# chenbinghui1/DSL

Hardware: AMD Instinct MI355X
Metric: imgs/sec training step, FCOS R50-FPN 1333x800 (higher is better)
Workload: dtype bf16; 1 GPU; FCOS R50-caffe-FPN supervised training step (BASELINE.json configs[1]), 2 x (3,800,1344) per GPU, synthetic COCO-shaped boxes, random-init weights; global_batch=2, parallelism=dp1, optimizer=SGD momentum 0.9 wd 1e-4

## Files before the change

dsl_amd/_lib.py:

```python
import ctypes as C
import os

import torch

HERE = os.path.dirname(os.path.abspath(__file__))
LIB_PATH = os.environ.get('DSL_HIP_LIB') or os.path.join(HERE, 'lib', 'libdsl_hip.so')
MAX_SEG = 5

if not os.path.exists(LIB_PATH):
    raise RuntimeError(
        f'{LIB_PATH} not found: the MI355X kernels are not built. Run `python -m dsl_amd.build` '
        '(needs hipcc); dsl_amd has no CPU or PyTorch fallback for its hot path.')
lib = C.CDLL(LIB_PATH)

I5 = C.c_int32 * MAX_SEG
F5 = C.c_float * MAX_SEG

CONV_RELU_OUT, CONV_RELU_IN, CONV_OUT_F32, CONV_MASK_FIRST, CONV_MASK_LAST, CONV_ADD_UPSAMPLE, \
    CONV_SMALL_C = 1, 2, 4, 8, 16, 32, 64
CONV_FP8 = 128
CONV_EPI_STAGED = 1 << 16
(OP_CONV, OP_WGRAD, OP_GN_FWD, OP_GN_BWD, OP_MAXPOOL, OP_SUM2X2, OP_COLSUM, OP_MEMSET, OP_PACK_IMAGE,
 OP_ASSIGN, OP_LOSS, OP_FORK, OP_JOIN, OP_WGRAD_GROUP, OP_RECORD, OP_WAIT) = range(1, 17)
OP_RLA = 17
OP_PACK_DGRAD = 18
OP_WGRAD_MULTI = 19
OP_PROF = 21
OP_QUANT_FP8, OP_QUANT_FP8_W, OP_FP8_COMB = 22, 23, 24
OP_FP8_PREP, OP_QUANT_FP8_DELAYED = 27, 28
OP_STEM_POOL = 25
OP_BNECK = 26
PROF_CLASSES = 8
MAX_MULTI = 16
SLOT_TAIL, SLOT_PREFIX = 13, 14
SLOT_PACKS = 15
SUMSQ_PARTS = 256
# ... 312 lines not shown
```

dsl_amd/csrc/conv.hip:

```cpp
#include <stdlib.h>
#include <algorithm>

#include <mutex>
#include <type_traits>
#include <vector>

#include "common.hpp"

namespace {

constexpr int BPX = 128;
constexpr int BK = 64;

struct ConvK {
  int nseg, n;
  int gh[DSL_MAX_SEG], gw[DSL_MAX_SEG], sh[DSL_MAX_SEG], sw[DSL_MAX_SEG];
  int dh[DSL_MAX_SEG], dw[DSL_MAX_SEG], ah[DSL_MAX_SEG], aw[DSL_MAX_SEG];
  int pxstart[DSL_MAX_SEG + 1];
  long long soff[DSL_MAX_SEG], doff[DSL_MAX_SEG], aoff[DSL_MAX_SEG];
  int cs, cd, ldd, lda, ldm, kh, kw, stride, pad, mode, os, flags;
  int lds;
  int ktiles, kc;
  int ident;
  int addfast;
// ... 10 lines not shown
  const uint16_t* addend;
  const uint16_t* mask;
  float* gnws;
  const uint16_t* gnx;
  const float* gngamma;
  const float* gnbeta;
  const float* gnstats;
};

#define CONV_HOT_PARAMS                                                                                                   \
  const uint16_t* h_wgt, const uint16_t* h_src, const int h_wrow, const int h_xcd_chunk, const int h_gx, const int h_gy, \
      const int h_splits, const int h_kt_per_split, const int h_ktiles, const int h_kc, const int h_kw, const int h_lds
#define CONV_HOT_ARGS(k) \
  (k).wgt, (k).src, (int)(k).wrow, (k).xcd_chunk, (k).gx, (k).gy, (k).splits, (k).kt_per_split, (k).ktiles, (k).kc, (k).kw, (k).lds

enum ConvGen { kGenV1 = 0, kGenGlds, kGenPipe, kGenPipeGn, kGenPipeSmallC, kGenF8, kNumConvGen };
struct ConvWaves { int wco, wpx; };
struct ConvTile {
  int bco, bpx, nst, occ;
  double eff;
  int prof;
  ConvWaves gen[kNumConvGen];
};
constexpr ConvTile kConvTiles[] = {
    {256, 192, 2, 1, 1.0,  1, {{}, {4, 2}, {4, 2}, {4, 2}, {},     {4, 2}}},
    {256, 128, 3, 1, 1.0,  2, {{}, {4, 2}, {4, 2}, {4, 2}, {},     {4, 2}}},
    {128, 256, 3, 1, 1.0,  2, {{}, {2, 4}, {2, 4}, {},     {},     {}}},
    {128, 128, 2, 2, 0.7,  0, {{}, {2, 2}, {2, 4}, {},     {},     {2, 4}}},
    {64,  256, 2, 2, 0.95, 2, {{}, {1, 4}, {1, 8}, {},     {1, 8}, {}}},
    {128, 64,  3, 2, 0.9,  2, {{}, {},     {2, 2}, {},     {},     {}}},
    {64,  64,  3, 3, 1.3,  2, {{}, {},     {1, 2}, {},     {},     {}}},
    {64,  128, 3, 2, 1.25, 2, {{}, {},     {1, 4}, {},     {},     {}}},
};
constexpr int kNumConvTiles = sizeof(kConvTiles) / sizeof(kConvTiles[0]);
constexpr size_t conv_lds_bytes(int bco, int bpx, int wpx, int nst, bool glds) {
  const size_t ring = (size_t)nst * (bco + bpx) * 128, stg = (size_t)32 * wpx * (bco * 4 + 16);
  return glds || ring > stg ? ring : stg;
}
constexpr size_t conv_lds_bytes(const ConvTile& t, int gen) { return conv_lds_bytes(t.bco, t.bpx, t.gen[gen].wpx, t.nst, gen == kGenGlds); }

__device__ __forceinline__ u32x4 relu_bf16x8(u32x4 v) {
#pragma unroll
  for (int i = 0; i < 4; ++i) {
    uint32_t w = v[i];
    uint32_t neg = (w >> 15) & 0x00010001u;
    v[i] = w & ~(neg * 0xffffu);
  }
// ... 32 lines not shown
  for (int s = 1; s < DSL_MAX_SEG; ++s) {
    const bool in = s < p.nseg && gp >= p.pxstart[s];
    ps = in ? p.pxstart[s] : ps;
    gh = in ? p.gh[s] : gh;
    gw = in ? p.gw[s] : gw;
    sh = in ? p.sh[s] : sh;
    sw = in ? p.sw[s] : sw;
    soff = in ? (int)p.soff[s] : soff;
  }
  const int q = gp - ps;
  const int hw = gh * gw;
  img = q / hw;
  const int rem = q - img * hw;
  y = rem / gw;
  x = rem - y * gw;
}

__device__ __forceinline__ void conv_epilogue4(const ConvK& p, long long dpix, long long apix, int co, float v[4]) {
  const bool out_f32 = (p.flags & DSL_CONV_OUT_F32) != 0;
  const bool relu_out = (p.flags & DSL_CONV_RELU_OUT) != 0;
  const bool mask_first = (p.flags & DSL_CONV_MASK_FIRST) != 0 && p.mask != nullptr;
  const bool mask_last = (p.flags & DSL_CONV_MASK_LAST) != 0 && p.mask != nullptr;
  const bool has_mask = mask_first || mask_last;
  if (co + 3 < p.cd) {
    if (p.scale) {
      const f32x4 s4 = *reinterpret_cast<const f32x4*>(p.scale + co);
#pragma unroll
      for (int e = 0; e < 4; ++e) v[e] *= s4[e];
    }
    if (p.bias) {
// ... 602 lines not shown
template <int NMF, int NDS, int NVM>
__device__ __forceinline__ void sched_stage() {
#pragma unroll
  for (int i = 0; i < NMF; ++i) {
    __builtin_amdgcn_sched_group_barrier(0x008, 1, 0);
    if (i < NDS) __builtin_amdgcn_sched_group_barrier(0x100, 1, 0);
    if (i < NVM) __builtin_amdgcn_sched_group_barrier(0x020, 1, 0);
  }
}

#ifdef DSL_TRACE_BUILD
constexpr int kTraceIters = 40;
__device__ unsigned long long g_conv_trace[8 * kTraceIters * 8 + 8 * 16 + 8];
#endif

template <int BCO, int BPX, int WCO, int WPX, int CT, int PT, int RING, bool GNB = false, class Stamp>
__device__ __forceinline__ void conv_tile_epilogue(const ConvK& p, f32x16 (&acc)[CT][PT], unsigned char* smem, const int co0, const int px0,
                                                   const int totpx, Stamp&& stamp) {
  constexpr int T = 64 * WCO * WPX;
  const int tid = threadIdx.x, lane = tid & 63;
  const int wave = __builtin_amdgcn_readfirstlane(tid >> 6);
  const int wave_co = wave / WPX, wave_px = wave % WPX;
  const int frow = lane & 31, fhalf = lane >> 5;
  constexpr int ROWB = BCO * 4 + 16;
  constexpr int CPX = 32 * WPX;
  constexpr int GPR = BCO / 8;
  static_assert(CPX * ROWB <= conv_lds_bytes(BCO, BPX, WPX, RING / ((BCO + BPX) * 128), false) &&
                conv_lds_bytes(BCO, BPX, WPX, RING / ((BCO + BPX) * 128), false) <= 160 * 1024,
                "epilogue staging must fit in LDS: the host sizes the launch's LDS with conv_lds_bytes, max(ring, staging)");
  static_assert(T % GPR == 0, "a thread keeps its channel group across the staged rows");
  const Affine8 aff = conv_affine8(p, co0 + (tid % GPR) * 8);
  const EpiFast ef = conv_epi_fast(p, co0 + (tid % GPR) * 8);
  constexpr int ROWH = BCO * 2 + 16;
  static_assert((long long)BPX * ROWH <= (long long)RING, "the bf16 tile fits in the ring");
  if ((ef.on || (p.addfast == 2 && !(p.flags & DSL_CONV_OUT_F32))) && ef.has_add && p.addfast && !ef.mask_first && !(ef.mask_last && ef.relu) &&
      (p.cd & 7) == 0) {
    constexpr int RB = BCO * 2;
    constexpr int NCH = RB / 16;
    constexpr int FSH = RB >= 256 ? 0 : (RB == 128 ? 1 : 2);
    static_assert((long long)BPX * RB <= (long long)RING, "the dense bf16 tile fits in the ring");
    static_assert((BPX * RB) % (T * 16) == 0, "whole DMA instructions per wave");
    constexpr int NDMA = BPX * RB / (T * 16);
    lds_barrier();
    {
      const __amdgpu_buffer_rsrc_t rs_add = __builtin_amdgcn_make_buffer_rsrc((void*)p.addend, 0, 0x7fffffff, 0x00020000);
#pragma unroll
      for (int i = 0; i < NDMA; ++i) {
        const int off = (i * (T / 64) + wave) * 1024 + lane * 16;
        const int row = off / RB, slot = (off % RB) >> 4;
        const int c = slot ^ ((row >> FSH) & (NCH - 1));
// ... 57 lines not shown
            u32x4 r = *reinterpret_cast<const u32x4*>(smem + row * RB + ((cgp ^ ((row >> FSH) & (NCH - 1))) << 4));
            if (ef.mask_last) {
              const u32x4 mm = *reinterpret_cast<const u32x4*>(ef.mask + (long long)gp * ef.ldm);
#pragma unroll
              for (int e = 0; e < 4; ++e)
                r[e] &= (bflo(mm[e]) > 0.f ? 0xffffu : 0x8000u) | (bfhi(mm[e]) > 0.f ? 0xffff0000u : 0x80000000u);
            }
            *reinterpret_cast<u32x4*>(out + (long long)gp * p.ldd) = r;
          }
        }
      }
    }
    stamp(3);
    return;
  }
  if (ef.on && !(p.flags & DSL_CONV_EPI_STAGED) && !ef.has_add && !ef.mask_first && !(ef.mask_last && ef.relu) && (p.cd & 7) == 0) {
    lds_barrier();
#pragma unroll
    for (int ct = 0; ct < CT; ++ct)
#pragma unroll
      for (int g = 0; g < 4; ++g) {
        const int col = wave_co * (32 * CT) + ct * 32 + 8 * g + 4 * fhalf;
        const bool in = co0 + col + 3 < p.cd;
        const f32x4 sc = (ef.has_scale && in) ? *reinterpret_cast<const f32x4*>(p.scale + co0 + col) : f32x4{1.f, 1.f, 1.f, 1.f};
        const f32x4 bi = (ef.has_bias && in) ? *reinterpret_cast<const f32x4*>(p.bias + co0 + col) : f32x4{0.f, 0.f, 0.f, 0.f};
#pragma unroll
        for (int pt = 0; pt < PT; ++pt) {
          float v[4];
#pragma unroll
          for (int j = 0; j < 4; ++j) {
            v[j] = acc[ct][pt][4 * g + j];
// ... 229 lines not shown
        f32x4 o = {acc[ct][pt][4 * g], acc[ct][pt][4 * g + 1], acc[ct][pt][4 * g + 2], acc[ct][pt][4 * g + 3]};
        *reinterpret_cast<f32x4*>(smem + (wave_px * 32 + frow) * ROWB + col * 4) = o;
      }
  };
  static_assert(PT <= 4, "slab dispatch");
#pragma nounroll
  for (int pt = 0; pt < PT; ++pt) {
    lds_barrier();
    stamp(1 + 3 * pt);
    if (pt == 0) stage_slab(std::integral_constant<int, 0>{});
    else if (pt == 1) stage_slab(std::integral_constant<int, (PT > 1 ? 1 : 0)>{});
    else if (pt == 2) stage_slab(std::integral_constant<int, (PT > 2 ? 2 : 0)>{});
    else stage_slab(std::integral_constant<int, (PT > 3 ? 3 : 0)>{});
    lds_barrier();
    stamp(2 + 3 * pt);
    if (ef.on && aff.full) {
      constexpr int NIT = CPX * GPR / T;
      static_assert(CPX * GPR % T == 0, "whole items per thread");
      const int pl0 = tid / GPR;
      const unsigned char* rd = smem + pl0 * ROWB + (tid % GPR) * 32;
#pragma nounroll
      for (int n_ = 0; n_ < NIT; ++n_) {
        const int pl = pl0 + n_ * (T / GPR);
        const int gp = px0 + (pl >> 5) * (32 * PT) + pt * 32 + (pl & 31);
        if (gp < totpx)
          conv_epilogue8_fast(ef, aff, gp, *reinterpret_cast<const f32x4*>(rd + n_ * (T / GPR) * ROWB),
                              *reinterpret_cast<const f32x4*>(rd + n_ * (T / GPR) * ROWB + 16));
      }
      stamp(3 + 3 * pt);
      continue;
    }
#pragma nounroll
    for (int id = tid; id < CPX * GPR; id += T) {
      const int pl = id / GPR, cg = id - pl * GPR;
      const int gp = px0 + (pl >> 5) * (32 * PT) + pt * 32 + (pl & 31);
      const int co = co0 + cg * 8;
      if (gp >= totpx || co >= p.cd) continue;
      const f32x4 lo = *reinterpret_cast<const f32x4*>(smem + pl * ROWB + cg * 32);
      const f32x4 hi = *reinterpret_cast<const f32x4*>(smem + pl * ROWB + cg * 32 + 16);
      float v[8] = {lo[0], lo[1], lo[2], lo[3], hi[0], hi[1], hi[2], hi[3]};
#ifdef DSL_ABLATE_BUILD
      if ((p.dbg & 512) && v[0] != 12345.678f) continue;
#endif
      long long dpix, apix;
      conv_out_index(p, gp, dpix, apix);
      conv_epilogue8a(p, dpix, apix, co, v, aff);
    }
    stamp(3 + 3 * pt);
  }
}

template <int BCO, int BPX, int WCO, int WPX, int NST, bool SMC = false, bool GNB = false>
__global__ __launch_bounds__(64 * WCO * WPX) void conv_pipe_kernel(CONV_HOT_PARAMS, const ConvK p) {
  extern __shared__ __attribute__((aligned(16))) unsigned char smem[];
  constexpr int T = 64 * WCO * WPX;
  constexpr int RPP = T / 8;
  constexpr int WPASS = BCO / RPP, XPASS = BPX / RPP;
  constexpr int TILE_W = BCO * 128;
  constexpr int STAGE = (BCO + BPX) * 128;
  constexpr int PT = BPX / WPX / 32;
  constexpr int CT = BCO / WCO / 32;
  constexpr int HB = 1;
  static_assert(BCO == WCO * CT * 32 && CT >= 1, "cout tiles per wave");
  static_assert(BCO % RPP == 0 && BPX % RPP == 0 && (BPX / WPX) % 32 == 0, "tile/thread mismatch");

  const int tid = threadIdx.x, lane = tid & 63;
  const int wave = __builtin_amdgcn_readfirstlane(tid >> 6);
// ... 7 lines not shown
  const int rem_t = wi - bz * (h_gx * h_gy);
  const int by = rem_t / h_gx;
  const int co0 = (rem_t - by * h_gx) * BCO;
  const int px0 = by * BPX;
  const int dt = tid, dwave = wave;
  const int lrow = dt >> 3;
  const int chunk = (dt & 7) ^ ((dt >> 4) & 7);

  const unsigned margin = (unsigned)(h_kw * h_lds * 2);
  const __amdgpu_buffer_rsrc_t rs_src =
      __builtin_amdgcn_make_buffer_rsrc((void*)(reinterpret_cast<const unsigned char*>(h_src) - margin), 0, 0x7fffffff, 0x00020000);
  const __amdgpu_buffer_rsrc_t rs_wgt = __builtin_amdgcn_make_buffer_rsrc((void*)h_wgt, 0, 0x7fffffff, 0x00020000);

  const int kt0 = bz * h_kt_per_split;
#ifdef DSL_ABLATE_BUILD
  const int kt1 = (p.dbg & 8) ? kt0 + 1 : min(kt0 + h_kt_per_split, h_ktiles);
#else
  const int kt1 = min(kt0 + h_kt_per_split, h_ktiles);
#endif
  const unsigned w_voff = (unsigned)(lrow * h_wrow + chunk * 8) * 2u;
  const unsigned w_pass = (unsigned)(RPP * h_wrow) * 2u;
  unsigned w_soff = (unsigned)(co0 * h_wrow + kt0 * BK) * 2u;
#pragma unroll
  for (int i = 0; i < WPASS; ++i) {
#ifdef DSL_ABLATE_BUILD
    if (p.dbg & 2) continue;
#endif
    __builtin_amdgcn_raw_ptr_buffer_load_lds(rs_wgt, (lptr_t)(smem + (i * RPP + dwave * 8) * 128), 16, w_voff, w_soff + i * w_pass, 0, 0);
  }
  __builtin_amdgcn_sched_barrier(0);

  const int totpx = p.pxstart[p.nseg];
  int cidx = kt0 % h_kc;
  int tap_r = (kt0 / h_kc) / h_kw, tap_s = (kt0 / h_kc) % h_kw;

  unsigned r_cur[XPASS], r_step[XPASS], r_mask[XPASS];
  int r_y[XPASS], r_x[XPASS], r_hw[XPASS];
#pragma unroll
  for (int i = 0; i < XPASS; ++i) {
    const int gp = px0 + lrow + RPP * i;
    int img, y, x, sh, sw, soff;
    const bool ok = gp < totpx;
    decode_pixel_src(p, ok ? gp : 0, img, y, x, sh, sw, soff);
    if (SMC) {
      r_y[i] = ok ? y * p.stride - p.pad : -100000;
      r_x[i] = x * p.stride - p.pad;
      r_hw[i] = (sh << 16) | sw;
      r_cur[i] = (unsigned)((soff + img * sh * sw + r_y[i] * sw + r_x[i]) * 16) + margin;
      r_step[i] = r_mask[i] = 0;
      continue;
    }
    const int row0 = p.mode == 0 ? y * p.stride - p.pad : y + p.pad;
    const int col0 = p.mode == 0 ? x * p.stride - p.pad : x + p.pad - (h_kw - 1);
    unsigned m = 0;
    for (int r = 0; r < p.kh; ++r) {
      const int sy = p.mode == 0 ? row0 + r : row0 - r;
      if (ok && (unsigned)sy < (unsigned)sh) m |= 1u << r;
// ... 8 lines not shown
    const unsigned base = (unsigned)((soff + img * sh * sw + row0 * sw + col0) * h_lds + chunk * 8) * 2u + margin;
    r_cur[i] = base + (unsigned)tap_r * r_step[i];
  }

  constexpr int LPT = WPASS + XPASS;
  constexpr int P0 = (LPT + 1) / 3;
  constexpr int P1 = P0 + (LPT - P0 + 1) / 2;
  int kt_next = kt0;
  unsigned t_sel = (1u << tap_r) | (0x100u << tap_s);
  unsigned t_soff = (unsigned)((p.mode == 0 ? tap_s : h_kw - 1 - tap_s) * h_lds * 2 + cidx * 128);
  unsigned t_wv = w_voff;
  int c_left = h_kc - cidx;
  unsigned r_v[XPASS];
#pragma unroll
  for (int i = 0; i < XPASS; ++i) r_v[i] = (r_mask[i] & t_sel) == t_sel ? r_cur[i] : 0x80000000u;
  auto pieces_of = [&](auto lo_c, auto hi_c, const unsigned ld_off, auto skipw_c) {
    constexpr int LO = decltype(lo_c)::value, HI = decltype(hi_c)::value;
    constexpr bool SKIPW = decltype(skipw_c)::value;
    unsigned char* stage = smem + ld_off;
    const bool live = kt_next < kt1;
    const unsigned s_off = t_soff;
    const unsigned wv = t_wv;
    int s_tr = 0, s_ts = 0;
    bool s_ok = false;
    if (SMC) {
      const int tap = kt_next * 8 + chunk;
      s_tr = tap / h_kw;
      s_ts = tap - s_tr * h_kw;
      s_ok = live && tap < p.kh * h_kw;
    }
// ... 13 lines not shown
          v = r_v[j];
          so = s_off;
        }
        __builtin_amdgcn_raw_ptr_buffer_load_lds(rs_src, (lptr_t)(stage + TILE_W + (j * RPP + dwave * 8) * 128), 16, v, so, 0, 0);
      } else if (!SKIPW) {
        const int i = j - XPASS;
        __builtin_amdgcn_raw_ptr_buffer_load_lds(rs_wgt, (lptr_t)(stage + (i * RPP + dwave * 8) * 128), 16, wv,
                                                 w_soff + i * w_pass, 0, 0);
      }
    }
    if (HI == LPT) {
      ++kt_next;
      w_soff += BK * 2;
      if (--c_left != 0) {
        t_soff += 128;
      } else {
        c_left = h_kc;
        const bool s_wrap = tap_s + 1 == h_kw;
        tap_s = s_wrap ? 0 : tap_s + 1;
        if (s_wrap) {
          ++tap_r;
#pragma unroll
          for (int i = 0; i < XPASS; ++i) r_cur[i] += r_step[i];
        }
        t_sel = (1u << tap_r) | (0x100u << tap_s);
        t_soff = (unsigned)((p.mode == 0 ? tap_s : h_kw - 1 - tap_s) * h_lds * 2);
#pragma unroll
        for (int i = 0; i < XPASS; ++i) r_v[i] = (r_mask[i] & t_sel) == t_sel ? r_cur[i] : 0x80000000u;
      }
      if (__builtin_expect(kt_next >= kt1, 0)) {
// ... 189 lines not shown
      if (gp >= totpx) continue;
      float* row = p.ws + ((long long)bz * totpx + gp) * p.cd_pad;
#pragma unroll
      for (int ct = 0; ct < CT; ++ct)
#pragma unroll
        for (int g = 0; g < 4; ++g) {
          const int co = co0 + wave_co * (32 * CT) + ct * 32 + 8 * g + 4 * (lane >> 5);
          f32x4 o = {acc[ct][pt][4 * g], acc[ct][pt][4 * g + 1], acc[ct][pt][4 * g + 2], acc[ct][pt][4 * g + 3]};
          *reinterpret_cast<f32x4*>(row + co) = o;
        }
    }
    return;
  }

#ifdef DSL_TRACE_BUILD
  conv_tile_epilogue<BCO, BPX, WCO, WPX, CT, PT, NST * STAGE, GNB>(p, acc, smem, co0, px0, totpx, [&](int i_) { TRE(i_); });
#else
  conv_tile_epilogue<BCO, BPX, WCO, WPX, CT, PT, NST * STAGE, GNB>(p, acc, smem, co0, px0, totpx, [](int) {});
#endif
#ifdef DSL_TRACE_BUILD
  trace_dump();
#endif
#undef TRE
}

typedef int v8i32 __attribute__((ext_vector_type(8)));
template <int BCO, int BPX, int WCO, int WPX, int NST>
__global__ __launch_bounds__(64 * WCO * WPX) void conv_f8_kernel(CONV_HOT_PARAMS, const ConvK p) {
  constexpr bool SMC = false;
  extern __shared__ __attribute__((aligned(16))) unsigned char smem[];
  constexpr int T = 64 * WCO * WPX;
  constexpr int RPP = T / 8;
  constexpr int WPASS = BCO / RPP, XPASS = BPX / RPP;
// ... 209 lines not shown
          const int co = co0 + wave_co * 64 + ct * 32 + 8 * g + 4 * (lane >> 5);
          f32x4 o = {acc[ct][pt][4 * g], acc[ct][pt][4 * g + 1], acc[ct][pt][4 * g + 2], acc[ct][pt][4 * g + 3]};
          *reinterpret_cast<f32x4*>(row + co) = o;
        }
    }
    return;
  }

  conv_tile_epilogue<BCO, BPX, WCO, WPX, 2, PT, NST * STAGE>(p, acc, smem, co0, px0, totpx, [](int) {});
}

}

namespace {
const char* const kConvGenNames[kNumConvGen] = {"conv_gemm_kernel", "conv_glds_kernel", "conv_pipe_kernel", "conv_pipe_kernel (backward GroupNorm records)",
                                                "conv_pipe_kernel (SMALL_C)", "conv_f8_kernel"};

inline bool conv_v2_only(const dsl_conv_desc* d) { return d->mode == 1 && d->stride > 1; }

double conv_cost_us(const ConvTile& c, long long px, int cd_pad, int ktiles, int sp, bool out_f32) {
  const long long wgs = (long long)(cd_pad / c.bco) * ((px + c.bpx - 1) / c.bpx) * sp;
  const long long slots = 256LL * c.occ;
  const long long rounds = (wgs + slots - 1) / slots;
  const long long per_cu = (wgs + 255) / 256;
  const double share = (double)(per_cu < c.occ ? per_cu : c.occ);
  const double mfma = c.bco * c.bpx / 32.0, dma = (c.bco + c.bpx) * 128 / 54.0;
  const double tile = share * (1.15 * (mfma > dma ? mfma : dma) + 0.5 * (mfma > dma ? dma : mfma)) * c.eff;
  const double fixed = (1000.0 + 0.05 * c.bco * c.bpx) * (share > 1.0 ? share / 2.0 : share);
  const int kt = (ktiles + sp - 1) / sp;
  double t = 4.0 + rounds * (kt * tile + fixed) / 2240.0;
  t += (double)px * cd_pad * (out_f32 ? 4 : 2) / 4.0e6;
  if (sp > 1) t += 3.0 + 2.0 * sp * px * cd_pad * 4 / 4.0e6;
  return t;
}

bool conv_cfg_ok(const dsl_conv_desc* d, int c, bool every_gen = true) {
  const ConvTile& T = kConvTiles[c];
  const int force = (d->flags >> 8) & 15;
  if (d->cd_pad % T.bco || (force >= 1 && force <= kNumConvTiles && force - 1 != c)) return false;
  if (conv_v2_only(d) && !T.gen[kGenGlds].wco) return false;
  if (!every_gen) return true;
  return !(d->gn_x && !T.gen[kGenPipeGn].wco) && !((d->flags & DSL_CONV_SMALL_C) && !T.gen[kGenPipeSmallC].wco) &&
         !((d->flags & DSL_CONV_FP8) && !T.gen[kGenF8].wco);
}

void conv_choose(const dsl_conv_desc* d, long long px, int ktiles, int* pick_out, int* splits_out) {
  const bool smallc = (d->flags & DSL_CONV_SMALL_C) != 0, fp8 = (d->flags & DSL_CONV_FP8) != 0;
  const int force = (d->flags >> 8) & 15;
  const int force_split = (d->flags >> 12) & 15;
  int pick = -1, splits = 1;
  long long src_px = 0;
  for (int sg = 0; sg < d->nseg; ++sg) src_px += (long long)d->n * d->sh[sg] * d->sw[sg];
  const long long lds_ = d->lds > 0 ? d->lds : d->cs;
  const bool dma_ok = conv_v2_only(d) || (d->kh <= 8 && d->kw <= 8 && src_px * lds_ * 2 + (long long)d->kw * lds_ * 2 < 0x7fff0000LL);
  const bool smallc_pipe = smallc && d->cd_pad % 64 == 0;
  const bool v1_only = ((smallc && !smallc_pipe) || (d->flags & DSL_CONV_RELU_IN) || !dma_ok) && !fp8;
  const bool out_f32 = (d->flags & DSL_CONV_OUT_F32) != 0;
  double best = 1e300;
  for (int pass = 0; pass < 2 && pick < 0 && !v1_only && force != 15 && (pass == 0 || force_split > 1); ++pass)
    for (int c = 0; c < kNumConvTiles; ++c) {
      if (!conv_cfg_ok(d, c, pass == 0)) continue;
      for (int sp = 1; sp <= (pass ? 1 : 16); ++sp) {
        if (sp > 1 && (smallc || fp8 || d->gn_ws)) break;
        if (sp > 1 && (!d->workspace || sp > ktiles / 2 || (size_t)sp * px * d->cd_pad * 4 > d->workspace_bytes)) break;
        if (!pass && force_split > 1 && sp != force_split) continue;
        const double t = conv_cost_us(kConvTiles[c], px, d->cd_pad, ktiles, sp, out_f32);
        if (t < best) { best = t; pick = c; splits = sp; }
      }
    }
  *pick_out = pick;
  *splits_out = splits;
}

double conv_real_cin(const dsl_conv_desc* d) {
  return (d->flags & DSL_CONV_SMALL_C) ? 3.0 : (double)(d->cs_real > 0 ? d->cs_real : d->cs);
}
double conv_algo_flops(const dsl_conv_desc* d, long long px) {
  return 2.0 * px * (double)d->cd * d->kh * d->kw * conv_real_cin(d);
// ... 19 lines not shown
}

int conv_ktiles(const dsl_conv_desc* d) {
  if (d->flags & DSL_CONV_SMALL_C) return (d->kh * d->kw + 7) / 8;
  return d->kh * d->kw * (d->cs / ((d->flags & DSL_CONV_FP8) ? 128 : 64));
}

bool conv_gn_ok(const dsl_conv_desc* d) {
  if (d->nseg < 1 || d->nseg > DSL_MAX_SEG) return false;
  if (d->flags & (DSL_CONV_SMALL_C | DSL_CONV_OUT_F32 | DSL_CONV_ADD_UPSAMPLE | DSL_CONV_RELU_IN)) return false;
  if ((d->flags & DSL_CONV_FP8) && d->gn_x) return false;
  if (d->cs % 64 || d->cd % 8 || d->cd_pad % 64 || d->os != 1 || d->addend) return false;
  if (d->mask && ((d->flags & DSL_CONV_MASK_FIRST) || ((d->flags & DSL_CONV_MASK_LAST) && (d->flags & DSL_CONV_RELU_OUT)))) return false;
  for (int s = 0; s < d->nseg; ++s)
    if (d->gh[s] != d->dh[s] || d->gw[s] != d->dw[s]) return false;
  if (conv_v2_only(d)) return false;
  dsl_conv_desc t = *d;
  t.gn_ws = (void*)1;
  int pick, splits;
  conv_choose(&t, conv_pixels(d), conv_ktiles(d), &pick, &splits);
  if (pick < 0 || splits != 1) return false;
  if (d->gn_x && (!kConvTiles[pick].gen[kGenPipeGn].wco || d->ldd != d->cd)) return false;
  return true;
}

int conv_validate(const dsl_conv_desc* d) {
  DSL_CHECK(d != nullptr, "dsl_conv2d: null descriptor");
  DSL_CHECK(d->nseg >= 1 && d->nseg <= DSL_MAX_SEG, "dsl_conv2d: nseg=%d out of range", d->nseg);
  DSL_CHECK(d->src && d->wgt && d->dst, "dsl_conv2d: null tensor pointer");
  const bool fp8 = (d->flags & DSL_CONV_FP8) != 0;
  if (d->flags & DSL_CONV_SMALL_C)
// ... 58 lines not shown
  k.ktiles = conv_ktiles(d);
  k.kc = (d->flags & DSL_CONV_SMALL_C) ? 1 : d->cs / (fp8 ? 128 : 64);
  k.wrow = (long long)k.ktiles * (fp8 ? 128 : BK);
  k.src = (const uint16_t*)d->src; k.wgt = (const uint16_t*)d->wgt; k.dst = d->dst;
  k.scale = d->scale; k.bias = d->bias;
  k.addend = (const uint16_t*)d->addend; k.mask = (const uint16_t*)d->mask;
  k.gnws = (float*)d->gn_ws;
  if (d->gn_ws && d->gn_x) { k.gnx = (const uint16_t*)d->gn_x; k.gngamma = d->gn_gamma; k.gnbeta = d->gn_beta; k.gnstats = d->gn_stats; }
}

int conv_plan(const dsl_conv_desc* d, ConvK& k, dsl_conv_plan& p) {
  const int px = k.pxstart[k.nseg];
  int pick, splits;
  conv_choose(d, px, k.ktiles, &pick, &splits);
  memset(&p, 0, sizeof(p));
  p.cfg = pick; p.splits = splits; p.ident = k.ident; p.addfast = k.addfast;
  if (pick < 0) {
    p.kernel = kGenV1; p.bco = (d->cd_pad % 128 == 0) ? 128 : 64; p.bpx = BPX; p.threads = 256;
    p.grid[0] = d->cd_pad / p.bco; p.grid[1] = (px + BPX - 1) / BPX; p.grid[2] = 1;
    p.lds_bytes = 2 * (size_t)(p.bco + BPX) * BK * 2;
    return 0;
  }
  const ConvTile& T = kConvTiles[pick];
  p.kernel = (d->flags & DSL_CONV_FP8) ? kGenF8 : conv_v2_only(d) ? kGenGlds : k.gnx ? kGenPipeGn
             : ((d->flags & DSL_CONV_SMALL_C) && T.gen[kGenPipeSmallC].wco) ? kGenPipeSmallC : kGenPipe;
  const ConvWaves W = T.gen[p.kernel];
  if (p.kernel == kGenF8) DSL_CHECK(W.wco, "dsl_conv2d: no fp8 kernel for this shape (tile config %d)", pick);
  DSL_CHECK(W.wco, "dsl_conv2d: no %s for tile config %d", kConvGenNames[p.kernel], pick);
  p.bco = T.bco; p.bpx = T.bpx; p.threads = 64 * W.wco * W.wpx;
  p.lds_bytes = conv_lds_bytes(T, p.kernel);
  p.workspace_bytes = splits > 1 ? (size_t)splits * px * d->cd_pad * 4 : 0;
  k.splits = splits;
  k.kt_per_split = (k.ktiles + splits - 1) / splits;
  k.cd_pad = d->cd_pad;
  k.ws = (float*)d->workspace;
  k.gx = d->cd_pad / T.bco;
  k.gy = (px + T.bpx - 1) / T.bpx;
  k.xcd_chunk = (int)(((unsigned)k.gx * k.gy * splits + 7) / 8);
  if (p.kernel == kGenGlds) { p.grid[0] = k.gx; p.grid[1] = k.gy; p.grid[2] = splits; }
// ... 46 lines not shown
    prof = dsl_prof_begin(p.kernel == kGenV1 ? 2 : kConvTiles[p.cfg].prof, conv_algo_flops(d, px), st, conv_algo_bytes(d, px));
  if (p.kernel == kGenV1) {
    const bool smallc = (d->flags & DSL_CONV_SMALL_C) != 0;
    if (p.bco == 128) smallc ? conv_run<conv_gemm_kernel<128, true>>(p, lds, st, k) : conv_run<conv_gemm_kernel<128, false>>(p, lds, st, k);
    else smallc ? conv_run<conv_gemm_kernel<64, true>>(p, lds, st, k) : conv_run<conv_gemm_kernel<64, false>>(p, lds, st, k);
  } else {
    conv_dispatch(p.cfg, p.kernel, [&](auto row) {
      constexpr ConvTile T = kConvTiles[decltype(row)::value];
      if (p.kernel == kGenPipe) conv_run<conv_pipe_kernel<CONV_TILE_ARGS(T, kGenPipe)>>(p, lds, st, CONV_HOT_ARGS(k), k);
      if constexpr (T.gen[kGenGlds].wco != 0)
        if (p.kernel == kGenGlds) conv_run<conv_glds_kernel<CONV_TILE_ARGS(T, kGenGlds)>>(p, lds, st, k);
      if constexpr (T.gen[kGenPipeGn].wco != 0)
        if (p.kernel == kGenPipeGn) conv_run<conv_pipe_kernel<CONV_TILE_ARGS(T, kGenPipeGn), false, true>>(p, lds, st, CONV_HOT_ARGS(k), k);
      if constexpr (T.gen[kGenPipeSmallC].wco != 0)
        if (p.kernel == kGenPipeSmallC) conv_run<conv_pipe_kernel<CONV_TILE_ARGS(T, kGenPipeSmallC), true>>(p, lds, st, CONV_HOT_ARGS(k), k);
      if constexpr (T.gen[kGenF8].wco != 0)
        if (p.kernel == kGenF8) conv_run<conv_f8_kernel<CONV_TILE_ARGS(T, kGenF8)>>(p, lds, st, CONV_HOT_ARGS(k), k);
    });
  }
  dsl_prof_end(prof, st);
  if (p.splits > 1) {
    const long long total = (long long)px * (k.cd_pad / 4);
    int blocks = (int)((total + 255) / 256);
    if (blocks > 4096) blocks = 4096;
    hipLaunchKernelGGL(conv_splitk_epilogue_kernel, dim3(blocks), dim3(256), 0, st, k.ws, px, k.cd_pad, k.cd, k.splits, k);
  }
  DSL_LAUNCH_CHECK(kConvGenNames[p.kernel]);
  return 0;
}
}
// ... 37 lines not shown
```

dsl_amd/engine.py:

```python
import ctypes as C
import os

import torch

from . import _lib as L
from . import ops
from .head_loss import FcosLossPlan
from .params import STAGE_BLOCKS, STAGE_PLANES
from .tuning import skip_items, tune, tune_int

DEFER_SLOTS = 144

BF = torch.bfloat16


class OpList:
    def __init__(self):
        self.items, self.keep, self.arr = [], [], None

    def _add(self, kind, desc=None, i=(), p=(), l=()):
        o = L.Op()
        o.kind = kind
        for k, v in enumerate(i):
            o.i[k] = int(v)
# ... 518 lines not shown
                                         pad=1 if spec is None else spec.pad)
        return self._wg_buf(need)

    def _wg_buf(self, need, name='wg_ws'):
        ws = self.bufs.get(name)
        if ws is None or ws.numel() < need:
            ws = torch.empty(max(need, 96 << 20), dtype=torch.uint8, device=self.dev)
            self.bufs.setdefault(name + '_old', []).append(self.bufs.get(name))
            self.bufs[name] = ws
        return ws

    def _dgrad(self, name, dy, dst, n, dy_hw, dst_hw, *, cs, cd, k, stride, pad, os=1, addend=None, mask=None,
               mask_first=False, mask_last=False, cs_real=0, wptr=None, cd_pad=None, ldd=None, lda=None, ldm=None):
        st = self.store
        f = (L.CONV_MASK_FIRST if mask_first else 0) | (L.CONV_MASK_LAST if mask_last else 0)
        grid = dy_hw if os > 1 else dst_hw
        return ops.conv_desc(dy, wptr if wptr is not None else st.wT_ptr(name), dst, n=n, grid=grid, src_hw=dy_hw, dst_hw=dst_hw,
                             cs=cs, cd=cd, cd_pad=cd_pad or cd, ldd=ldd or cd, kh=k, kw=k, stride=stride, pad=pad, mode=1, os=os,
                             flags=f, addend=addend, lda=lda or cd, mask=mask, ldm=ldm or cd, workspace=self.conv_ws,
                             cs_real=cs_real)

    def _build_backward(self):
        st, N, ls = self.store, self.N, self.level_sizes
        lp = self.lossplan
        reg = st.train_regions
        M = self.M
        SIDE = tune('side') != '0'
        GROUP_LAST = True
        TAIL_SLOTS = tune_int('tail_slots')
        GROUP = True
# ... 365 lines not shown
```

dsl_amd/engine_rla.py:

```python
import ctypes as C

import torch

from . import _lib as L
from . import ops
from .params import RLA_C, RLA_PAD, STAGE_BLOCKS, STAGE_PLANES
from .tuning import tune, tune_int

BF = torch.bfloat16


def _rla_op(ol, kind, p=(), i=(), f=(), rows=0, side=False):
    d = L.RlaDesc()
    d.kind = kind
    for k, v in enumerate(p):
        d.p[k] = v if isinstance(v, int) else (0 if v is None else v.data_ptr())
    for k, v in enumerate(i):
        d.i[k] = int(v)
    for k, v in enumerate(f):
        d.f[k] = float(v)
    d.rows = int(rows)
    d._keep = [v for v in p if not isinstance(v, int)]
    ol._add(L.OP_RLA, d, i=(0, 0, 0, 0, 0, 0, int(side)))
    return d
# ... 91 lines not shown
    if split_open:
        f.join(plan.BR)
    plan._keep_rla = getattr(plan, '_keep_rla', [])


def build_backward(plan, buckets, SIDE):
    st, N = plan.store, plan.N
    cv = st.convs
    g32 = lambda name: st.t32_ptr(name, st.grad)
    bn_g = lambda bn, leaf: st.t32_ptr('bn_train.' + leaf, st.grad) + st.bn_train_off[bn][0] * 4
    bn_p = lambda bn, leaf: st.t32_ptr('bn_train.' + leaf) + st.bn_train_off[bn][0] * 4
    bn_f = lambda bn, leaf: st.frozen.data_ptr() + (st.frozen_regions['bn_train.' + leaf][0] + st.bn_train_off[bn][0]) * 4
    from .engine import OpList
    TAIL = tune('rla_tail') != '0'
    BSPLIT = tune('rla_split_bwd')
    S2_CLASSES = True
    BB = plan.BR

    def br_ws(d_):
        d_.workspace, d_.workspace_bytes = L.ptr(plan.conv_ws_br), plan.conv_ws_br.numel()
        return d_
    gh_next = None
    for s_ in (3, 2, 1):
        ol = OpList()
        blks = [b for b in plan.rla_blocks if b['stage'] == s_]
        planes, c4 = blks[0]['planes'], blks[0]['c4']
        co, rc = cv[f'backbone.conv_outs.{s_}'], cv[f'backbone.recurrent_convs.{s_}']
        gx = plan.g_stage[s_]
        g3, g2, g1, g_co, g_rc, post = [], [], [], [], [], []
        bsplit = str(s_) in BSPLIT
        groups = [(0, (N + 1) // 2, 0), ((N + 1) // 2, N, BB)] if bsplit else [(0, N, 0)]
# ... 160 lines not shown
```

dsl_amd/tuning.py:

```python
import os

DEFAULTS = {
    'side': '1',
    'pipe_prefix': '1',
    'img_split': '234',
    'bneck_fwd': '2',
    'img_split_bwd': '23',
    'tower_slots': '72',
    'tail_slots': '192',
    'rla_split': '123',
    'rla_tail': '1',
    'rla_split_bwd': '',
    'check_backward_grad': '0',
    'skip': '',
    'lib.wgrad_slots': '128',
    'lib.stream_probe': '1',
    'lib.comm_queue': '1',
    'lib.rla_tail_form': '0',
    'lib.debug_sync': '0',
    'lib.skip_kinds': '0',
}

_values = dict(DEFAULTS)
_parsed = False
# ... 47 lines not shown
```

include/dsl_hip.h:

```cpp
#ifndef DSL_HIP_H
#define DSL_HIP_H
#include <stddef.h>
#include <stdint.h>

#ifdef __cplusplus
extern "C" {
#endif

#define DSL_MAX_SEG 5
#define DSL_MAX_GROUP 8

int dsl_version(void);
const char* dsl_last_error(void);
int dsl_set_option(const char* name, int value);
int dsl_get_option(const char* name, int* value);

enum {
  DSL_CONV_RELU_OUT = 1,
  DSL_CONV_RELU_IN = 2,
  DSL_CONV_OUT_F32 = 4,
  DSL_CONV_MASK_FIRST = 8,
  DSL_CONV_MASK_LAST = 16,
  DSL_CONV_ADD_UPSAMPLE = 32,
  DSL_CONV_SMALL_C = 64,
  DSL_CONV_FP8 = 128,
  DSL_CONV_EPI_STAGED = 1 << 16
};

typedef struct dsl_conv_desc {
  int32_t nseg, n;
  int32_t gh[DSL_MAX_SEG], gw[DSL_MAX_SEG];
  int32_t sh[DSL_MAX_SEG], sw[DSL_MAX_SEG];
  int32_t dh[DSL_MAX_SEG], dw[DSL_MAX_SEG];
  int32_t ah[DSL_MAX_SEG], aw[DSL_MAX_SEG];
  int32_t cs;
  int32_t cd;
  int32_t cd_pad;
  int32_t ldd, lda, ldm;
  int32_t kh, kw, stride, pad, mode, os, flags;
  const void* src;
  const void* wgt;
// ... 458 lines not shown
```

Baseline: 459.1 imgs/s.

## Add parity-class data-gradient kernel for stride-2 3x3 convolutions

Adds a new conv_pipe_kernel variant for the data gradient of stride-2 3x3 convolutions. Output pixels are reordered into four parity classes so that each tile iterates only over the kernel taps that land on real (non-zero-stuffed) input positions, which removes the wasted MACs of the transposed-conv formulation. It is enabled by default through a new dgrad_parity tune key and flag, and it replaces the older S2_CLASSES split in the RLA backward. In exchange it disables split-K and the fast epilogue paths for these convs and adds per-tile parity decode arithmetic.

```diff
diff --git a/dsl_amd/_lib.py b/dsl_amd/_lib.py
--- a/dsl_amd/_lib.py
+++ b/dsl_amd/_lib.py
@@ -20,6 +20,7 @@
     CONV_SMALL_C = 1, 2, 4, 8, 16, 32, 64
 CONV_FP8 = 128
 CONV_EPI_STAGED = 1 << 16
+CONV_DGRAD_PARITY = 1 << 17
 (OP_CONV, OP_WGRAD, OP_GN_FWD, OP_GN_BWD, OP_MAXPOOL, OP_SUM2X2, OP_COLSUM, OP_MEMSET, OP_PACK_IMAGE,
  OP_ASSIGN, OP_LOSS, OP_FORK, OP_JOIN, OP_WGRAD_GROUP, OP_RECORD, OP_WAIT) = range(1, 17)
 OP_RLA = 17
diff --git a/dsl_amd/csrc/conv.hip b/dsl_amd/csrc/conv.hip
--- a/dsl_amd/csrc/conv.hip
+++ b/dsl_amd/csrc/conv.hip
@@ -48,7 +48,7 @@
 #define CONV_HOT_ARGS(k) \
   (k).wgt, (k).src, (int)(k).wrow, (k).xcd_chunk, (k).gx, (k).gy, (k).splits, (k).kt_per_split, (k).ktiles, (k).kc, (k).kw, (k).lds
 
-enum ConvGen { kGenV1 = 0, kGenGlds, kGenPipe, kGenPipeGn, kGenPipeSmallC, kGenF8, kNumConvGen };
+enum ConvGen { kGenV1 = 0, kGenGlds, kGenPipe, kGenPipeGn, kGenPipeSmallC, kGenF8, kGenPipeSdg, kNumConvGen };
 struct ConvWaves { int wco, wpx; };
 struct ConvTile {
   int bco, bpx, nst, occ;
@@ -57,14 +57,14 @@
   ConvWaves gen[kNumConvGen];
 };
 constexpr ConvTile kConvTiles[] = {
-    {256, 192, 2, 1, 1.0,  1, {{}, {4, 2}, {4, 2}, {4, 2}, {},     {4, 2}}},
-    {256, 128, 3, 1, 1.0,  2, {{}, {4, 2}, {4, 2}, {4, 2}, {},     {4, 2}}},
-    {128, 256, 3, 1, 1.0,  2, {{}, {2, 4}, {2, 4}, {},     {},     {}}},
-    {128, 128, 2, 2, 0.7,  0, {{}, {2, 2}, {2, 4}, {},     {},     {2, 4}}},
-    {64,  256, 2, 2, 0.95, 2, {{}, {1, 4}, {1, 8}, {},     {1, 8}, {}}},
-    {128, 64,  3, 2, 0.9,  2, {{}, {},     {2, 2}, {},     {},     {}}},
-    {64,  64,  3, 3, 1.3,  2, {{}, {},     {1, 2}, {},     {},     {}}},
-    {64,  128, 3, 2, 1.25, 2, {{}, {},     {1, 4}, {},     {},     {}}},
+    {256, 192, 2, 1, 1.0,  1, {{}, {4, 2}, {4, 2}, {4, 2}, {},     {4, 2}, {}}},
+    {256, 128, 3, 1, 1.0,  2, {{}, {4, 2}, {4, 2}, {4, 2}, {},     {4, 2}, {}}},
+    {128, 256, 3, 1, 1.0,  2, {{}, {2, 4}, {2, 4}, {},     {},     {},     {}}},
+    {128, 128, 2, 2, 0.7,  0, {{}, {2, 2}, {2, 4}, {},     {},     {2, 4}, {2, 4}}},
+    {64,  256, 2, 2, 0.95, 2, {{}, {1, 4}, {1, 8}, {},     {1, 8}, {},     {}}},
+    {128, 64,  3, 2, 0.9,  2, {{}, {},     {2, 2}, {},     {},     {},     {}}},
+    {64,  64,  3, 3, 1.3,  2, {{}, {},     {1, 2}, {},     {},     {},     {1, 2}}},
+    {64,  128, 3, 2, 1.25, 2, {{}, {},     {1, 4}, {},     {},     {},     {1, 4}}},
 };
 constexpr int kNumConvTiles = sizeof(kConvTiles) / sizeof(kConvTiles[0]);
 constexpr size_t conv_lds_bytes(int bco, int bpx, int wpx, int nst, bool glds) {
@@ -127,6 +127,47 @@
   const int rem = q - img * hw;
   y = rem / gw;
   x = rem - y * gw;
+}
+
+__device__ __forceinline__ void sdg_starts(const ConvK& p, int (&st)[5], int (&ni)[2], int (&nj)[2]) {
+  const int H = p.gh[0], W = p.gw[0];
+  ni[0] = (H + 1) >> 1; ni[1] = H >> 1;
+  nj[0] = (W + 1) >> 1; nj[1] = W >> 1;
+  st[0] = 0;
+#pragma unroll
+  for (int c = 0; c < 4; ++c) st[c + 1] = st[c] + p.n * ni[c >> 1] * nj[c & 1];
+}
+__device__ __forceinline__ void sdg_decode(const ConvK& p, int gp, int& img, int& y, int& x) {
+  int st[5], ni[2], nj[2];
+  sdg_starts(p, st, ni, nj);
+  const int py = gp >= st[2], px = py ? gp >= st[3] : gp >= st[1];
+  const int q = gp - (py ? (px ? st[3] : st[2]) : (px ? st[1] : 0));
+  const int h2 = py ? ni[1] : ni[0], w2 = px ? nj[1] : nj[0];
+  const int hw = h2 * w2;
+  img = q / hw;
+  const int rem = q - img * hw;
+  const int i = rem / w2;
+  y = 2 * i + py;
+  x = 2 * (rem - i * w2) + px;
+}
+__device__ __forceinline__ unsigned sdg_tile_taps(const ConvK& p, int px0, int px1) {
+  int st[5], ni[2], nj[2];
+  sdg_starts(p, st, ni, nj);
+  unsigned m = 0;
+#pragma unroll
+  for (int r = 0; r < 3; ++r)
+#pragma unroll
+    for (int s = 0; s < 3; ++s) {
+      const int c = 2 * ((r + p.pad) & 1) + ((s + p.pad) & 1);
+      int lo = st[0], hi = st[1];
+#pragma unroll
+      for (int k = 1; k < 4; ++k) {
+        lo = c == k ? st[k] : lo;
+        hi = c == k ? st[k + 1] : hi;
+      }
+      if (lo < px1 && hi > px0) m |= 1u << (r * 3 + s);
+    }
+  return m;
 }
 
 __device__ __forceinline__ void conv_epilogue4(const ConvK& p, long long dpix, long long apix, int co, float v[4]) {
@@ -759,7 +800,7 @@
 __device__ unsigned long long g_conv_trace[8 * kTraceIters * 8 + 8 * 16 + 8];
 #endif
 
-template <int BCO, int BPX, int WCO, int WPX, int CT, int PT, int RING, bool GNB = false, class Stamp>
+template <int BCO, int BPX, int WCO, int WPX, int CT, int PT, int RING, bool GNB = false, bool SDG = false, class Stamp>
 __device__ __forceinline__ void conv_tile_epilogue(const ConvK& p, f32x16 (&acc)[CT][PT], unsigned char* smem, const int co0, const int px0,
                                                    const int totpx, Stamp&& stamp) {
   constexpr int T = 64 * WCO * WPX;
@@ -778,7 +819,7 @@
   const EpiFast ef = conv_epi_fast(p, co0 + (tid % GPR) * 8);
   constexpr int ROWH = BCO * 2 + 16;
   static_assert((long long)BPX * ROWH <= (long long)RING, "the bf16 tile fits in the ring");
-  if ((ef.on || (p.addfast == 2 && !(p.flags & DSL_CONV_OUT_F32))) && ef.has_add && p.addfast && !ef.mask_first && !(ef.mask_last && ef.relu) &&
+  if (!SDG && (ef.on || (p.addfast == 2 && !(p.flags & DSL_CONV_OUT_F32))) && ef.has_add && p.addfast && !ef.mask_first && !(ef.mask_last && ef.relu) &&
       (p.cd & 7) == 0) {
     constexpr int RB = BCO * 2;
     constexpr int NCH = RB / 16;
@@ -866,7 +907,7 @@
     stamp(3);
     return;
   }
-  if (ef.on && !(p.flags & DSL_CONV_EPI_STAGED) && !ef.has_add && !ef.mask_first && !(ef.mask_last && ef.relu) && (p.cd & 7) == 0) {
+  if (!SDG && ef.on && !(p.flags & DSL_CONV_EPI_STAGED) && !ef.has_add && !ef.mask_first && !(ef.mask_last && ef.relu) && (p.cd & 7) == 0) {
     lds_barrier();
 #pragma unroll
     for (int ct = 0; ct < CT; ++ct)
@@ -1126,7 +1167,7 @@
     else stage_slab(std::integral_constant<int, (PT > 3 ? 3 : 0)>{});
     lds_barrier();
     stamp(2 + 3 * pt);
-    if (ef.on && aff.full) {
+    if (!SDG && ef.on && aff.full) {
       constexpr int NIT = CPX * GPR / T;
       static_assert(CPX * GPR % T == 0, "whole items per thread");
       const int pl0 = tid / GPR;
@@ -1155,14 +1196,20 @@
       if ((p.dbg & 512) && v[0] != 12345.678f) continue;
 #endif
       long long dpix, apix;
-      conv_out_index(p, gp, dpix, apix);
+      if constexpr (SDG) {
+        int img, y, x;
+        sdg_decode(p, gp, img, y, x);
+        dpix = apix = ((long long)img * p.dh[0] + y) * p.dw[0] + x;
+      } else {
+        conv_out_index(p, gp, dpix, apix);
+      }
       conv_epilogue8a(p, dpix, apix, co, v, aff);
     }
     stamp(3 + 3 * pt);
   }
 }
 
-template <int BCO, int BPX, int WCO, int WPX, int NST, bool SMC = false, bool GNB = false>
+template <int BCO, int BPX, int WCO, int WPX, int NST, bool SMC = false, bool GNB = false, bool SDG = false>
 __global__ __launch_bounds__(64 * WCO * WPX) void conv_pipe_kernel(CONV_HOT_PARAMS, const ConvK p) {
   extern __shared__ __attribute__((aligned(16))) unsigned char smem[];
   constexpr int T = 64 * WCO * WPX;
@@ -1200,13 +1247,24 @@
 
   const int kt0 = bz * h_kt_per_split;
 #ifdef DSL_ABLATE_BUILD
-  const int kt1 = (p.dbg & 8) ? kt0 + 1 : min(kt0 + h_kt_per_split, h_ktiles);
+  const int kt1_all = (p.dbg & 8) ? kt0 + 1 : min(kt0 + h_kt_per_split, h_ktiles);
 #else
-  const int kt1 = min(kt0 + h_kt_per_split, h_ktiles);
+  const int kt1_all = min(kt0 + h_kt_per_split, h_ktiles);
 #endif
+  unsigned sdg_taps = 0;
+  int sdg_tap0 = 0, sdg_nk = 0;
+  if constexpr (SDG) {
+    sdg_taps = sdg_tile_taps(p, px0, min(px0 + BPX, p.pxstart[1]));
+    sdg_nk = __builtin_popcount(sdg_taps) * h_kc;
+    sdg_tap0 = __builtin_ctz(sdg_taps | 0x100u);
+    sdg_taps &= sdg_taps - 1;
+  }
+  const int kt1 = SDG ? sdg_nk : kt1_all;
   const unsigned w_voff = (unsigned)(lrow * h_wrow + chunk * 8) * 2u;
   const unsigned w_pass = (unsigned)(RPP * h_wrow) * 2u;
   unsigned w_soff = (unsigned)(co0 * h_wrow + kt0 * BK) * 2u;
+  const unsigned w_row0 = w_soff;
+  if constexpr (SDG) w_soff += (unsigned)(sdg_tap0 * h_kc * (BK * 2));
 #pragma unroll
   for (int i = 0; i < WPASS; ++i) {
 #ifdef DSL_ABLATE_BUILD
@@ -1219,6 +1277,10 @@
   const int totpx = p.pxstart[p.nseg];
   int cidx = kt0 % h_kc;
   int tap_r = (kt0 / h_kc) / h_kw, tap_s = (kt0 / h_kc) % h_kw;
+  if constexpr (SDG) {
+    tap_r = sdg_tap0 / 3;
+    tap_s = sdg_tap0 - tap_r * 3;
+  }
 
   unsigned r_cur[XPASS], r_step[XPASS], r_mask[XPASS];
   int r_y[XPASS], r_x[XPASS], r_hw[XPASS];
@@ -1227,6 +1289,14 @@
     const int gp = px0 + lrow + RPP * i;
     int img, y, x, sh, sw, soff;
     const bool ok = gp < totpx;
+    if constexpr (SDG) {
+      sdg_decode(p, ok ? gp : 0, img, y, x);
+      r_y[i] = ok ? ((y + p.pad) << 16) | (x + p.pad) : -1;
+      r_cur[i] = (unsigned)((img * p.sh[0] * p.sw[0]) * h_lds + chunk * 8) * 2u + margin;
+      r_x[i] = r_hw[i] = 0;
+      r_step[i] = r_mask[i] = 0;
+      continue;
+    }
     decode_pixel_src(p, ok ? gp : 0, img, y, x, sh, sw, soff);
     if (SMC) {
       r_y[i] = ok ? y * p.stride - p.pad : -100000;
@@ -1265,6 +1335,16 @@
   unsigned r_v[XPASS];
 #pragma unroll
   for (int i = 0; i < XPASS; ++i) r_v[i] = (r_mask[i] & t_sel) == t_sel ? r_cur[i] : 0x80000000u;
+  auto sdg_rv = [&](int i) -> unsigned {
+    const int ty = (r_y[i] >> 16) - tap_r, tx = (r_y[i] & 0xffff) - tap_s;
+    const bool in = r_y[i] >= 0 && (ty | tx) >= 0 && !((ty | tx) & 1) && (ty >> 1) < p.sh[0] && (tx >> 1) < p.sw[0];
+    return in ? r_cur[i] + (unsigned)(((ty >> 1) * p.sw[0] + (tx >> 1)) * h_lds) * 2u : 0x80000000u;
+  };
+  if constexpr (SDG) {
+    t_soff = 0;
+#pragma unroll
+    for (int i = 0; i < XPASS; ++i) r_v[i] = sdg_rv(i);
+  }
   auto pieces_of = [&](auto lo_c, auto hi_c, const unsigned ld_off, auto skipw_c) {
     constexpr int LO = decltype(lo_c)::value, HI = decltype(hi_c)::value;
     constexpr bool SKIPW = decltype(skipw_c)::value;
@@ -1308,6 +1388,16 @@
       w_soff += BK * 2;
       if (--c_left != 0) {
         t_soff += 128;
+      } else if constexpr (SDG) {
+        c_left = h_kc;
+        const int tap = __builtin_ctz(sdg_taps | 0x100u);
+        sdg_taps &= sdg_taps - 1;
+        tap_r = tap / 3;
+        tap_s = tap - tap_r * 3;
+        w_soff = w_row0 + (unsigned)(tap * h_kc * (BK * 2));
+        t_soff = 0;
+#pragma unroll
+        for (int i = 0; i < XPASS; ++i) r_v[i] = sdg_rv(i);
       } else {
         c_left = h_kc;
         const bool s_wrap = tap_s + 1 == h_kw;
@@ -1527,9 +1617,9 @@
   }
 
 #ifdef DSL_TRACE_BUILD
-  conv_tile_epilogue<BCO, BPX, WCO, WPX, CT, PT, NST * STAGE, GNB>(p, acc, smem, co0, px0, totpx, [&](int i_) { TRE(i_); });
+  conv_tile_epilogue<BCO, BPX, WCO, WPX, CT, PT, NST * STAGE, GNB, SDG>(p, acc, smem, co0, px0, totpx, [&](int i_) { TRE(i_); });
 #else
-  conv_tile_epilogue<BCO, BPX, WCO, WPX, CT, PT, NST * STAGE, GNB>(p, acc, smem, co0, px0, totpx, [](int) {});
+  conv_tile_epilogue<BCO, BPX, WCO, WPX, CT, PT, NST * STAGE, GNB, SDG>(p, acc, smem, co0, px0, totpx, [](int) {});
 #endif
 #ifdef DSL_TRACE_BUILD
   trace_dump();
@@ -1769,9 +1859,19 @@
 
 namespace {
 const char* const kConvGenNames[kNumConvGen] = {"conv_gemm_kernel", "conv_glds_kernel", "conv_pipe_kernel", "conv_pipe_kernel (backward GroupNorm records)",
-                                                "conv_pipe_kernel (SMALL_C)", "conv_f8_kernel"};
-
-inline bool conv_v2_only(const dsl_conv_desc* d) { return d->mode == 1 && d->stride > 1; }
+                                                "conv_pipe_kernel (SMALL_C)", "conv_f8_kernel", "conv_pipe_kernel (parity-class data gradient)"};
+
+inline bool conv_sdg(const dsl_conv_desc* d) {
+  if (!(d->flags & DSL_CONV_DGRAD_PARITY) || d->mode != 1 || d->stride != 2 || d->kh != 3 || d->kw != 3 || d->nseg != 1 || d->os != 1) return false;
+  if (d->flags & (DSL_CONV_SMALL_C | DSL_CONV_FP8 | DSL_CONV_RELU_IN | DSL_CONV_ADD_UPSAMPLE | DSL_CONV_OUT_F32)) return false;
+  if (d->gn_ws || d->gh[0] != d->dh[0] || d->gw[0] != d->dw[0] || d->cd % 8 || d->dh[0] > 16000 || d->dw[0] > 16000) return false;
+  const long long lds_ = d->lds > 0 ? d->lds : d->cs;
+  if (((long long)d->n * d->sh[0] * d->sw[0] + 3) * lds_ * 2 >= 0x7fff0000LL) return false;
+  if ((long long)d->n * d->gh[0] * d->gw[0] >= 0x7fff0000LL) return false;
+  const int force = (d->flags >> 8) & 15;
+  return force == 0 || force > kNumConvTiles || (force != 15 && kConvTiles[force - 1].gen[kGenPipeSdg].wco != 0);
+}
+inline bool conv_v2_only(const dsl_conv_desc* d) { return d->mode == 1 && d->stride > 1 && !conv_sdg(d); }
 
 double conv_cost_us(const ConvTile& c, long long px, int cd_pad, int ktiles, int sp, bool out_f32) {
   const long long wgs = (long long)(cd_pad / c.bco) * ((px + c.bpx - 1) / c.bpx) * sp;
@@ -1794,6 +1894,7 @@
   const int force = (d->flags >> 8) & 15;
   if (d->cd_pad % T.bco || (force >= 1 && force <= kNumConvTiles && force - 1 != c)) return false;
   if (conv_v2_only(d) && !T.gen[kGenGlds].wco) return false;
+  if (conv_sdg(d) && !T.gen[kGenPipeSdg].wco) return false;
   if (!every_gen) return true;
   return !(d->gn_x && !T.gen[kGenPipeGn].wco) && !((d->flags & DSL_CONV_SMALL_C) && !T.gen[kGenPipeSmallC].wco) &&
          !((d->flags & DSL_CONV_FP8) && !T.gen[kGenF8].wco);
@@ -1811,12 +1912,14 @@
   const bool smallc_pipe = smallc && d->cd_pad % 64 == 0;
   const bool v1_only = ((smallc && !smallc_pipe) || (d->flags & DSL_CONV_RELU_IN) || !dma_ok) && !fp8;
   const bool out_f32 = (d->flags & DSL_CONV_OUT_F32) != 0;
+  const bool sdg = conv_sdg(d);
+  if (sdg) ktiles = (ktiles + 3) / 4;
   double best = 1e300;
   for (int pass = 0; pass < 2 && pick < 0 && !v1_only && force != 15 && (pass == 0 || force_split > 1); ++pass)
     for (int c = 0; c < kNumConvTiles; ++c) {
       if (!conv_cfg_ok(d, c, pass == 0)) continue;
       for (int sp = 1; sp <= (pass ? 1 : 16); ++sp) {
-        if (sp > 1 && (smallc || fp8 || d->gn_ws)) break;
+        if (sp > 1 && (smallc || fp8 || d->gn_ws || sdg)) break;
         if (sp > 1 && (!d->workspace || sp > ktiles / 2 || (size_t)sp * px * d->cd_pad * 4 > d->workspace_bytes)) break;
         if (!pass && force_split > 1 && sp != force_split) continue;
         const double t = conv_cost_us(kConvTiles[c], px, d->cd_pad, ktiles, sp, out_f32);
@@ -1866,7 +1969,7 @@
   if (d->mask && ((d->flags & DSL_CONV_MASK_FIRST) || ((d->flags & DSL_CONV_MASK_LAST) && (d->flags & DSL_CONV_RELU_OUT)))) return false;
   for (int s = 0; s < d->nseg; ++s)
     if (d->gh[s] != d->dh[s] || d->gw[s] != d->dw[s]) return false;
-  if (conv_v2_only(d)) return false;
+  if (d->mode == 1 && d->stride > 1) return false;
   dsl_conv_desc t = *d;
   t.gn_ws = (void*)1;
   int pick, splits;
@@ -1955,6 +2058,8 @@
   int pick, splits;
   conv_choose(d, px, k.ktiles, &pick, &splits);
   memset(&p, 0, sizeof(p));
+  const bool sdg = pick >= 0 && conv_sdg(d);
+  if (sdg) k.ident = k.addfast = 0;
   p.cfg = pick; p.splits = splits; p.ident = k.ident; p.addfast = k.addfast;
   if (pick < 0) {
     p.kernel = kGenV1; p.bco = (d->cd_pad % 128 == 0) ? 128 : 64; p.bpx = BPX; p.threads = 256;
@@ -1963,7 +2068,7 @@
     return 0;
   }
   const ConvTile& T = kConvTiles[pick];
-  p.kernel = (d->flags & DSL_CONV_FP8) ? kGenF8 : conv_v2_only(d) ? kGenGlds : k.gnx ? kGenPipeGn
+  p.kernel = (d->flags & DSL_CONV_FP8) ? kGenF8 : sdg ? kGenPipeSdg : conv_v2_only(d) ? kGenGlds : k.gnx ? kGenPipeGn
              : ((d->flags & DSL_CONV_SMALL_C) && T.gen[kGenPipeSmallC].wco) ? kGenPipeSmallC : kGenPipe;
   const ConvWaves W = T.gen[p.kernel];
   if (p.kernel == kGenF8) DSL_CHECK(W.wco, "dsl_conv2d: no fp8 kernel for this shape (tile config %d)", pick);
@@ -2040,6 +2145,9 @@
         if (p.kernel == kGenPipeGn) conv_run<conv_pipe_kernel<CONV_TILE_ARGS(T, kGenPipeGn), false, true>>(p, lds, st, CONV_HOT_ARGS(k), k);
       if constexpr (T.gen[kGenPipeSmallC].wco != 0)
         if (p.kernel == kGenPipeSmallC) conv_run<conv_pipe_kernel<CONV_TILE_ARGS(T, kGenPipeSmallC), true>>(p, lds, st, CONV_HOT_ARGS(k), k);
+      if constexpr (T.gen[kGenPipeSdg].wco != 0)
+        if (p.kernel == kGenPipeSdg)
+          conv_run<conv_pipe_kernel<CONV_TILE_ARGS(T, kGenPipeSdg), false, false, true>>(p, lds, st, CONV_HOT_ARGS(k), k);
       if constexpr (T.gen[kGenF8].wco != 0)
         if (p.kernel == kGenF8) conv_run<conv_f8_kernel<CONV_TILE_ARGS(T, kGenF8)>>(p, lds, st, CONV_HOT_ARGS(k), k);
     });
diff --git a/dsl_amd/engine.py b/dsl_amd/engine.py
--- a/dsl_amd/engine.py
+++ b/dsl_amd/engine.py
@@ -556,6 +556,8 @@
                mask_first=False, mask_last=False, cs_real=0, wptr=None, cd_pad=None, ldd=None, lda=None, ldm=None):
         st = self.store
         f = (L.CONV_MASK_FIRST if mask_first else 0) | (L.CONV_MASK_LAST if mask_last else 0)
+        if k == 3 and stride == 2 and tune('dgrad_parity') != '0':
+            f |= L.CONV_DGRAD_PARITY
         grid = dy_hw if os > 1 else dst_hw
         return ops.conv_desc(dy, wptr if wptr is not None else st.wT_ptr(name), dst, n=n, grid=grid, src_hw=dy_hw, dst_hw=dst_hw,
                              cs=cs, cd=cd, cd_pad=cd_pad or cd, ldd=ldd or cd, kh=k, kw=k, stride=stride, pad=pad, mode=1, os=os,
diff --git a/dsl_amd/engine_rla.py b/dsl_amd/engine_rla.py
--- a/dsl_amd/engine_rla.py
+++ b/dsl_amd/engine_rla.py
@@ -129,7 +129,7 @@
     from .engine import OpList
     TAIL = tune('rla_tail') != '0'
     BSPLIT = tune('rla_split_bwd')
-    S2_CLASSES = True
+    S2_CLASSES = tune('dgrad_parity') == '0'
     BB = plan.BR
 
     def br_ws(d_):
diff --git a/dsl_amd/tuning.py b/dsl_amd/tuning.py
--- a/dsl_amd/tuning.py
+++ b/dsl_amd/tuning.py
@@ -8,6 +8,7 @@
     'img_split_bwd': '23',
     'tower_slots': '72',
     'tail_slots': '192',
+    'dgrad_parity': '1',
     'rla_split': '123',
     'rla_tail': '1',
     'rla_split_bwd': '',
diff --git a/include/dsl_hip.h b/include/dsl_hip.h
--- a/include/dsl_hip.h
+++ b/include/dsl_hip.h
@@ -24,7 +24,8 @@
   DSL_CONV_ADD_UPSAMPLE = 32,
   DSL_CONV_SMALL_C = 64,
   DSL_CONV_FP8 = 128,
-  DSL_CONV_EPI_STAGED = 1 << 16
+  DSL_CONV_EPI_STAGED = 1 << 16,
+  DSL_CONV_DGRAD_PARITY = 1 << 17
 };
 
 typedef struct dsl_conv_desc {
```

After: 460.8 imgs/s (median of 3 runs). No clear change (+0.4%).
